# bistromath/gr-ais

Hardware: AMD Instinct MI355X
Metric: complex MS/s through corr_est->msk_timing chain; corr_est %HBM roofline (higher is better)
Workload: dtype f32

## Files before the change

gr-ais_amd/csrc/aisx_common.h:

```cpp
#pragma once
#include <math.h>
#include <stdint.h>

#if defined(__HIPCC__)
#include <hip/hip_runtime.h>
#define AISX_DI __device__ __forceinline__
#define AISX_HD __host__ __device__ __forceinline__
#else
#define AISX_DI inline
#define AISX_HD inline
#endif

namespace aisx {

struct cf {
    float re, im;
};

AISX_HD cf mk(float re, float im)
{
    cf r;
    r.re = re;
    r.im = im;
    return r;
}
AISX_HD cf operator+(cf a, cf b) { return mk(a.re + b.re, a.im + b.im); }
AISX_HD cf operator-(cf a, cf b) { return mk(a.re - b.re, a.im - b.im); }
AISX_HD cf cconj(cf a) { return mk(a.re, -a.im); }

struct alignas(8) cf_a8 { float re, im; };
struct alignas(16) cf_a16 { float re0, im0, re1, im1; };
AISX_HD cf ld8(const cf* p)
{
    const cf_a8 v = *reinterpret_cast<const cf_a8*>(p);
    return mk(v.re, v.im);
}
AISX_HD void st8(cf* p, cf v)
{
    cf_a8 t;
    t.re = v.re;
    t.im = v.im;
    *reinterpret_cast<cf_a8*>(p) = t;
}
AISX_HD void ld16(const cf* p, cf& a, cf& b)
{
    const cf_a16 v = *reinterpret_cast<const cf_a16*>(p);
    a = mk(v.re0, v.im0);
    b = mk(v.re1, v.im1);
}
AISX_HD void st16(cf* p, cf a, cf b)
{
    cf_a16 t;
    t.re0 = a.re;
    t.im0 = a.im;
    t.re1 = b.re;
    t.im1 = b.im;
    *reinterpret_cast<cf_a16*>(p) = t;
}

AISX_HD cf cmul_exact(cf a, cf b) { return mk(a.re * b.re - a.im * b.im, a.re * b.im + a.im * b.re); }

AISX_HD cf cmul_fma(cf a, cf b)
{
    return mk(fmaf(-a.im, b.im, a.re * b.re), fmaf(a.im, b.re, a.re * b.im));
}
AISX_HD cf cmul_conj_fma(cf a, cf b)
{
    return mk(fmaf(a.im, b.im, a.re * b.re), fmaf(a.im, b.re, -(a.re * b.im)));
}

AISX_HD float mag2(cf a) { return a.re * a.re + a.im * a.im; }

AISX_HD float fdiv_rn(float a, float b)
{
#if defined(__HIP_DEVICE_COMPILE__)
    return __fdiv_rn(a, b);
#else
    return a / b;
#endif
}

AISX_HD float branchless_clip(float x, float clip)
{
    float x1 = fabsf(x + clip);
    float x2 = fabsf(x - clip);
    x1 -= x2;
    return 0.5f * x1;
}

AISX_HD int aisx_popc64(unsigned long long v) { return __builtin_popcountll(v); }

AISX_HD unsigned mmse_row_bits(float mu) { return __builtin_bit_cast(unsigned, fmaf(mu, 128.0f, 12582912.0f)); }
AISX_HD unsigned mmse_row(float mu) { return mmse_row_bits(mu) - 0x4B400000u; }
AISX_HD unsigned mmse_row_base(unsigned base, unsigned pitch) { return base - 0x400000u * pitch; }
AISX_HD unsigned mmse_row_off(float mu, unsigned pitch, unsigned row_base)
{
    return (mmse_row_bits(mu) & 0xFFFFFFu) * pitch + row_base;
}

AISX_HD unsigned ring_read_off(int sb, int adv, unsigned step, unsigned mask)
{
#if defined(__HIP_DEVICE_COMPILE__)
    unsigned r;
    asm("v_mad_u32_u24 %0, %1, %2, %3" : "=v"(r) : "v"(adv), "v"(step), "v"(sb));
    return r & mask;
#else
    return ((unsigned)sb + ((unsigned)adv & 0xFFFFFFu) * (step & 0xFFFFFFu)) & mask;
#endif
}

AISX_HD float fast_atan2f_tab(float y, float x, const float* tab)
{
    const float TAN_MAP_RES = 0.003921569f;
    const float PI_F = 3.14159265358979323846f, PI2_F = 1.57079632679489661923f;
    const float y_abs = fabsf(y), x_abs = fabsf(x);
    const bool ylt = y_abs < x_abs;
    const float z = fdiv_rn(ylt ? y_abs : x_abs, ylt ? x_abs : y_abs);
    float alpha = z * 255.0f;
    const int index = ((int)alpha) & 0xff;
    alpha -= (float)index;
    const float t0 = tab[index], t1 = tab[index + 1];
    float base_angle = t0 + (t1 - t0) * alpha;
    base_angle = (z < TAN_MAP_RES) ? z : base_angle;
    const bool xge = x >= 0.0f, yge = y >= 0.0f;
    const float a_h = xge ? (yge ? base_angle : -base_angle) : (yge ? (PI_F - base_angle) : (base_angle - PI_F));
    const float a_v = yge ? (xge ? (PI2_F - base_angle) : (PI2_F + base_angle))
                          : (xge ? (-PI2_F + base_angle) : (-PI2_F - base_angle));
    const float angle = (x_abs > y_abs) ? a_h : a_v;
    return ((y_abs > 0.0f) || (x_abs > 0.0f)) ? angle : 0.0f;
}

AISX_HD int fxpt_float_to_fixed(float x)
{
    const float PI = 3.14159265358979323846f, TAU = 2.0f * 3.14159265358979323846f, TWO_TO_THE_31 = 2147483648.0f;
    if (!(x >= -PI && x < PI)) {
        const int d = (int)floor((double)fdiv_rn(x, TAU) + 0.5);
        x -= (float)d * TAU;
    }
    const float RCP_PI = 0.318309886183790671538f;
    const float y = x * TWO_TO_THE_31;
    const float q = y * RCP_PI;
    return (int)fmaf(fmaf(-q, PI, y), RCP_PI, q);
}
AISX_HD void nco_sincos(float phase, const float* tab, float* s, float* c)
{
    const cf* T = reinterpret_cast<const cf*>(tab);
    const unsigned x = (unsigned)fxpt_float_to_fixed(phase);
    const unsigned xc = x + 0x40000000u;
    const cf es = ld8(T + (x >> 22)), ec = ld8(T + (xc >> 22));
    *s = es.re * (float)(x >> 1) + es.im;
    *c = ec.re * (float)(xc >> 1) + ec.im;
}

AISX_HD float nco_wrap(float ph)
{
    const float F_PI = 3.14159265358979323846f;
    const float TWO_PI = 2.0f * F_PI;
    const float u = ph + F_PI;
    float r;
    const float au = fabsf(u);
    if (au < TWO_PI)
        r = u;
    else if (au < 2.0f * TWO_PI)
        r = (u > 0.f) ? (u - TWO_PI) : (u + TWO_PI);
    else
        r = fmodf(u, TWO_PI);
    return r - F_PI;
}

AISX_HD float nco_wrap_small(float ph)
{
    const float F_PI = 3.14159265358979323846f;
    const float TWO_PI = 2.0f * F_PI;
    const float u = ph + F_PI;
    const float w = u - copysignf(TWO_PI, u);
    const float r = (fabsf(u) < TWO_PI) ? u : w;
    return r - F_PI;
}

#ifndef NCO_CKN
#define NCO_CKN 8
#endif
constexpr int NCO_CK = NCO_CKN;
static_assert(NCO_CK == 2 || NCO_CK == 4 || NCO_CK == 8, "checkpoints every 2, 4 or 8 items");
AISX_HD float nco_phase_step(float ph, float d, bool small) { return small ? nco_wrap_small(ph + d) : nco_wrap(ph + d); }

constexpr int NCO_TAB_FLOATS = 2048;

AISX_HD float cabs_f(cf a) { return (float)sqrt((double)a.re * (double)a.re + (double)a.im * (double)a.im); }

struct tag_rec {
    uint64_t offset;
    double value;
    int32_t key;
    int32_t chan;
};
enum { KEY_CORR_START = 0, KEY_PHASE_EST = 1, KEY_TIME_EST = 2, KEY_CORR_EST = 3 };

}
```

gr-ais_amd/csrc/k_msk.h:

```cpp
#pragma once
#include "aisx_common.h"

namespace aisx {

enum {
    MSK_ST_INTERP_RANGE = 1,
    MSK_ST_CARRY_OVERFLOW = 2,
    MSK_ST_TAGCARRY_OVERFLOW = 4,
    MSK_ST_OUT_FULL = 8,
    MSK_ST_TAGS_TRUNCATED = 16
};
constexpr int MSK_CTN_TRUNC = 0x40000000;
constexpr int MSK_CTN_WILD = 0x20000000;
constexpr int MSK_TAG_TRIPS = 6;

constexpr int MSK_T = 64;
constexpr int MSK_RING = 256;
constexpr int MSK_SLOTS = MSK_RING + 8;
constexpr int MSK_CHUNK = 64;
constexpr int MSK_OFF = 192;
constexpr int MSK_CARRY_MAX = 128;
constexpr int MSK_PAIRS_MAX = 16;
constexpr int MSK_TAPS_PITCH = 12;
constexpr int msk_lds_ring(int lpw) { return MSK_SLOTS * lpw * 8; }
constexpr int MSK_ZERO_ROW = 129;
constexpr int MSK_LDS_MMSE = ((130 * MSK_TAPS_PITCH * 4 + 511) / 512) * 512;
constexpr int MSK_TAGQ = 36;
#ifndef MSK_WAVES_LPW4
#define MSK_WAVES_LPW4 4
#endif
constexpr int msk_waves(int lpw) { return lpw >= 16 ? 64 / lpw : (lpw == 4 ? MSK_WAVES_LPW4 : 4); }
constexpr int msk_wg_channels(int lpw) { return msk_waves(lpw) * lpw; }
constexpr int MSK_STAGE = 32;
static_assert(MSK_STAGE >= 15 + MSK_PAIRS_MAX + 1, "a lock-step run and a general step between two flushes");
constexpr bool msk_staged(int lpw) { return lpw <= 8; }
constexpr int msk_lds_stage(int lpw) { return msk_staged(lpw) ? MSK_STAGE * lpw * 8 : 0; }
constexpr int msk_lds_ringoff(int lpw) { return msk_waves(lpw) * msk_lds_stage(lpw); }
constexpr int msk_lds_wave(int lpw) { return msk_lds_ring(lpw) + MSK_TAGQ * lpw * 8 + lpw * 8; }
constexpr int msk_lds_taboff(int lpw) { return msk_lds_ringoff(lpw) + msk_waves(lpw) * msk_lds_wave(lpw); }
constexpr int msk_lds_bytes(int lpw) { return msk_lds_taboff(lpw) + MSK_LDS_MMSE; }
static_assert(msk_lds_bytes(4) <= 160 * 1024 && msk_lds_bytes(8) <= 160 * 1024 && msk_lds_bytes(16) <= 160 * 1024 &&
              msk_lds_bytes(32) <= 160 * 1024 && msk_lds_bytes(64) <= 160 * 1024, "a workgroup's LDS");
static_assert(msk_lds_bytes(8) + 71680 <= 160 * 1024, "timing recovery + one correlator workgroup per CU");
constexpr int BT_T = 256;
constexpr int BT_SEG = BT_T * 8;

constexpr int MSKP_SMAX = 64;
enum { MSKP_KIND_NONE = 0, MSKP_KIND_NEXT = 1, MSKP_KIND_HANDOFF = 2 };
struct mskp_rst {
    int jA;
    int relA, relB;
    int q0, cap;
    int pad[3];
};
struct mskp_snap {
    int a;
    float mu, omega;
    int div;
    cf y;
    cf nl;
    int cur;
    int cnt;
};
struct mskp_res {
    mskp_snap end;
    cf ay, anl;
    int kind;
    int status;
};
struct mskp_piece {
    int out0, src0, cnt;
};
AISX_HD bool mskp_same_bits(cf a, cf b)
{
    unsigned ar, ai, br, bi;
    __builtin_memcpy(&ar, &a.re, 4);
    __builtin_memcpy(&ai, &a.im, 4);
    __builtin_memcpy(&br, &b.re, 4);
    __builtin_memcpy(&bi, &b.im, 4);
    return ar == br && ai == bi;
}

struct msk_ctag { int rel; float val; };

struct __attribute__((packed, aligned(8))) cf_pair { cf a, b; };

struct MskParams {
    int nchan;
    float d_sps, gain, gain_omega, limit;
    int osps;
    float* mu; float* omega; int* div;
    cf* dly1; cf* dly2; cf* diff1;
    unsigned long long* nread;
    const cf* in; long in_stride; int n;
    const cf* carry_in; cf* carry_out; const int* carry_len_in; int* carry_len_out; int carry_cap;
    int stream_mode; int gr_ninput; int gr_noutput;
    const msk_ctag* ct; const int* ct_n; int ct_cap;
    tag_rec* ctag_out; int* ctag_n_out; int ctag_cap;
    cf* syms; float* err; float* mu_out; long out_stride; int out_cap;
    int* produced; int* consumed; int* status;
    const float* mmse;
    int lds_tab_off;
    int lds_wave_stride, tq_stride, tq_private;
    int lds_ring_off;
    int sym_al16;
    int lpw;
    int inline_tags;
    int max_noutput;
    int ff;
    const int* nrst; const mskp_rst* rst; const mskp_res* res;
    mskp_piece* pieces; int* npieces;
    const int* ct_nc;
};

struct BitTailParams {
    int nchan;
    const cf* syms; long sym_stride;
    const int* produced;
    unsigned char* bits; long bit_stride;
    const cf* prev_sym_in; const unsigned char* prev_bit_in;
    cf* prev_sym_out; unsigned char* prev_bit_out;
    const float* atan_tab;
};

AISX_HD int msk_forecast(float d_sps, int noutput_items)
{
    return (int)ceil((noutput_items * d_sps * 2) + 3.0 * d_sps + 8u);
}

#ifdef MSK_EMU_STATS
extern long msk_stats[8];
#endif
template <class Ctx, bool AUX, bool OSPS2, int LPW, bool FFT = false>
AISX_DI void msk_body(Ctx& cx, const MskParams& p)
{
    static_assert(!FFT || (!AUX && !OSPS2), "the join build has no err / mu ports and osps == 1");
    constexpr int SLOT_B = LPW * 8;
    constexpr int SLOT_SH = LPW == 64 ? 9 : (LPW == 32 ? 8 : (LPW == 16 ? 7 : (LPW == 8 ? 6 : 5)));
    static_assert(LPW == 4 || LPW == 8 || LPW == 16 || LPW == 32 || LPW == 64, "channels per wave");
    typedef unsigned long long u64;
    static_assert(64 % LPW == 0, "whole waves");
    constexpr int NQ = 64 / LPW;
    constexpr int QS = MSK_CHUNK / NQ;
    const int wv = cx.tid() >> 6;
    const int l = cx.tid() & (LPW - 1);
    const int q = (cx.tid() & 63) / LPW;
    const bool owner = q == 0;
    const int cbase = cx.bx() * msk_wg_channels(LPW) + wv * LPW;
    const int c = cbase + l;
    const bool live = c < p.nchan;
    const int cc = live ? c : (p.nchan - 1);

    char* const lds0 = cx.lds();
    char* const lds = lds0 + p.lds_ring_off + wv * p.lds_wave_stride;
    cf* ring = (cf*)lds;
    float* mm = (float*)(lds0 + p.lds_tab_off);
    cf* myring = ring + l;

    for (int i = cx.tid(); i < 129 * 8; i += cx.nthreads())
        mm[(i >> 3) * MSK_TAPS_PITCH + (i & 7)] = p.mmse[i];
    if (cx.tid() < MSK_TAPS_PITCH)
        mm[MSK_ZERO_ROW * MSK_TAPS_PITCH + cx.tid()] = 0.f;
    if (cbase >= p.nchan) {
        cx.sync();
        return;
    }

    const float d_sps = p.d_sps;
    float d_mu = p.mu[cc], d_omega = p.omega[cc];
    int d_div = p.div[cc];
    cf last_interp = p.dly1[cc];
    cf d_dly_diff_1 = p.diff1[cc];
    cf prev_sq = cmul_exact(p.dly2[cc], p.dly2[cc]);
    const unsigned long long R = p.nread[cc];
    int status = 0;
    const int n = p.n;

    const cf* cin = p.carry_in + (long)cc * p.carry_cap;
    int pending = p.carry_len_in[cc];
    if (pending > MSK_CARRY_MAX)
        pending = MSK_CARRY_MAX;
    const int navail = pending + n;
    for (int q = -1; q < pending; q++) {
        const int slot = (q - pending + MSK_OFF) & (MSK_RING - 1);
        myring[slot * LPW] = cin[q + 1];
        if (slot < 8)
            myring[(MSK_RING + slot) * LPW] = cin[q + 1];
    }

    const msk_ctag* ctl = p.ct + (long)cc * p.ct_cap;
    int ntot = p.ct_n[cc];
    if (ntot & MSK_CTN_TRUNC)
        status |= MSK_ST_TAGS_TRUNCATED;
    const bool tame_tags = p.inline_tags && cx.ballot((ntot & MSK_CTN_WILD) != 0) == 0ull;
    ntot &= MSK_CTN_WILD - 1;
    if (ntot > p.ct_cap)
        ntot = p.ct_cap;
    typedef msk_ctag tq_ent;
    tq_ent* const tq = (tq_ent*)(lds + msk_lds_ring(LPW)) + (p.tq_private ? (cx.tid() & 63) : l);
    const int TQS = p.tq_stride;
    const int TQ_NONE = 0x7fffffff;
    int gq = 0;
    int qhead = 0, qn = 0;
    auto tq_fill = [&]() {
        if (qn > 0) {
            tq[0] = tq[(qn - 1) * TQS];
            qn = 1;
        }
        qhead = qn;
        while (qn < MSK_TAGQ && gq < ntot) {
            tq_ent t[4];
#pragma unroll
            for (int j = 0; j < 4; j++)
                t[j] = ctl[gq + j < ntot ? gq + j : ntot - 1];
#pragma unroll
            for (int j = 0; j < 4; j++) {
                if (qn < MSK_TAGQ && gq < ntot) {
                    gq++;
                    tq[qn * TQS] = t[j];
                    qn++;
                }
            }
        }
    };
    int fr_rel = TQ_NONE;
    float nt_val = 0.f;
    int nt_rel = 0x7fffffff;
    auto tq_front = [&]() {
        if (qhead >= qn && gq < ntot)
            tq_fill();
        if (qhead < qn) {
            const tq_ent e = tq[qhead * TQS];
            fr_rel = e.rel;
            nt_val = e.val;
        } else {
            fr_rel = TQ_NONE;
        }
    };
    auto tq_pop = [&]() {
        qhead++;
        tq_front();
    };
    tq_fill();

    constexpr bool FF = FFT;
    bool fin_saved = false;
    float fin_mu = 0.f, fin_omega = 0.f;
    int fin_div = 0, fin_status = 0;
    cf fin_interp = mk(0.f, 0.f), fin_diff = mk(0.f, 0.f);
    unsigned fin_worst = 0;
    int ffK = 0, ffnck = 0, cand = 0, candj = 0x7fffffff, ffnp = 0;
    int voff = 0;
    const mskp_rst* const ffrs = FF ? p.rst + (long)cc * MSKP_SMAX : nullptr;
    const mskp_res* const ffrr = FF ? p.res + (long)cc * MSKP_SMAX : nullptr;
    if (FF) {
        ffnck = p.ct_nc[cc];
        ffK = ffnck >= 0 ? p.nrst[cc] : 0;
        candj = ffK > 0 ? ffrs[0].jA + 1 + ffnck : 0x7fffffff;
    }

    char* const osym0 = (char*)(p.syms + (long)cbase * p.out_stride);
    char* const oerr0 = AUX && p.err ? (char*)(p.err + (long)cbase * p.out_stride) : nullptr;
    char* const omu0 = AUX && p.mu_out ? (char*)(p.mu_out + (long)cbase * p.out_stride) : nullptr;
    unsigned ob = (unsigned)((long)(cc - cbase) * p.out_stride) * 8u;
    constexpr bool STG = !AUX && !OSPS2 && msk_staged(LPW);
    constexpr unsigned FLQ = NQ < 8 ? NQ : 8;
    constexpr unsigned FL = 2 * FLQ;
    constexpr unsigned STG_MASK = (unsigned)((MSK_STAGE - 1) * SLOT_B);
    const unsigned obrow = ob;
    const unsigned stg_real = (unsigned)(wv * msk_lds_stage(LPW) + l * 8);
    const unsigned stg_spare = (unsigned)(p.lds_ring_off + wv * p.lds_wave_stride + p.lds_wave_stride - SLOT_B + l * 8);
    unsigned so = 0;
    unsigned nf = 0;
    struct alignas(8) cf8s { float re, im; };
    auto stage_put = [&](unsigned mask, unsigned base, cf v) {
        cf8s t;
        t.re = v.re;
        t.im = v.im;
        *(cf8s*)(lds0 + ((so & mask) | base)) = t;
        so += (unsigned)SLOT_B;
    };
    auto stage_get = [&](unsigned k) -> cf {
        const cf8s t = *(const cf8s*)(lds0 + ((((k & (unsigned)(MSK_STAGE - 1)) << SLOT_SH)) | stg_real));
        return mk(t.re, t.im);
    };
    auto flush_syms = [&]() {
        if constexpr (STG) {
            if (cx.ballot((so >> SLOT_SH) - nf >= FL) == 0ull)
                return;
            cx.wave_sync();
            while (cx.ballot((so >> SLOT_SH) - nf >= FL) != 0ull) {
                if ((so >> SLOT_SH) - nf >= FL) {
                    const unsigned k0 = nf + 2u * (unsigned)q;
                    if ((NQ <= 8 || (unsigned)q < FLQ) && !fin_saved) {
                        const cf a = stage_get(k0), b = stage_get(k0 + 1u);
                        cf* dst = (cf*)(osym0 + obrow) + k0;
                        if (p.sym_al16) {
                            st16(dst, a, b);
                        } else {
                            st8(dst, a);
                            st8(dst + 1, b);
                        }
                    }
                    nf += FL;
                }
            }
            cx.wave_sync();
        }
    };

    int base = 0, ototal = 0;
    int iidx = 0, oidx = 0;
    int ninp = 0, noutput = 0;
// ... 128 lines not shown
            ffnp++;
            moved = true;
            dcnt += r.end.cnt;
            oidx_w += r.end.cnt;
            while (p.max_noutput > 0 && oidx_w >= nout_w) {
                oidx_w -= nout_w;
                otot_w += nout_w;
                nout_w = p.max_noutput;
                crossed = true;
            }
            a_new = r.end.a;
            mu_new = r.end.mu;
            om_new = r.end.omega;
            div_new = r.end.div;
            yv = r.end.y;
            nlv = r.end.nl;
            cur_new = r.end.cur;
            status |= r.status;
            cand++;
            candj = cand < ffK ? ffrs[cand].jA + 1 + ffnck : 0x7fffffff;
            if (r.kind == MSKP_KIND_NEXT && cand < ffK)
                continue;
            break;
        }
        if (!moved)
            return false;
        if constexpr (STG) {
            if (owner) {
                for (unsigned kk = nf; kk < (so >> SLOT_SH); kk++)
                    st8((cf*)(osym0 + obrow) + kk, stage_get(kk));
            }
            nf = (so >> SLOT_SH) + (unsigned)dcnt;
            so += (unsigned)dcnt << SLOT_SH;
        }
        ob += (unsigned)dcnt * 8u;
        d_mu = mu_new;
        d_omega = om_new;
        d_div = div_new;
        last_interp = yv;
        prev_sq = cmul_exact(yv, yv);
        d_dly_diff_1 = nlv;
        gq = cur_new + ffnck;
        if (gq > ntot)
            gq = ntot;
        qn = 0;
        qhead = 0;
        tq_fill();
        const int q_new = a_new + pending;
        tq_front();
        if (crossed) {
            ototal = otot_w;
            base = (fr_rel != TQ_NONE && fr_rel < q_new) ? fr_rel : q_new;
            setup_round();
        } else {
            nt_rel = (fr_rel != TQ_NONE && fr_rel - base < ninp) ? fr_rel - base : 0x7fffffff;
        }
        iidx = q_new - base;
        oidx = oidx_w;
        const int v_new = loaded_s - MSK_CHUNK + 1;
        voff = a_new - v_new;
        sb = (v_new + MSK_OFF) * SLOT_B;
        {
            const int slot0 = (loaded_s - MSK_CHUNK + MSK_OFF) & (MSK_RING - 1);
            constexpr int SH = Ctx::wave_lds_coherent ? 1 : NQ;
            for (int sh = 0; sh < SH; sh++) {
                const int k0 = ((Ctx::wave_lds_coherent ? q : sh) * QS);
                cf t[QS];
#pragma unroll
                for (int k = 0; k < QS; k++) {
                    const int sr = loaded_s - MSK_CHUNK + k0 + k + voff;
                    t[k] = mk(0.f, 0.f);
                    if (sr >= 0 && sr < n)
                        t[k] = myin[sr];
                }
#pragma unroll
                for (int k = 0; k < QS; k++) {
                    myring[(slot0 + k0 + k) * LPW] = t[k];
                    if (slot0 == 0 && k0 + k < 8)
                        myring[(MSK_RING + k0 + k) * LPW] = t[k];
                }
            }
            if (more) {
                const int s0 = landed * MSK_CHUNK + q * QS + voff;
#pragma unroll
                for (int k = 0; k < QS; k++) {
                    r[k] = mk(0.f, 0.f);
                    if (s0 + k < n && s0 + k >= 0)
                        r[k] = myin[s0 + k];
                }
            }
        }
        tag_trig = (int)0x80000000;
        fast_lim = (int)0x80000000;
        return true;
    };
    auto events = [&](const int PAR) -> int {
        if (!(oidx < noutput && iidx < ninp)) {
            base += iidx;
            ototal += oidx;
            const bool progress = iidx > 0;
            if (!p.stream_mode || !progress)
                done = true;
            else
                setup_round();
        }
        if (done)
            return EV_PARK;
        const int spos = sb >> SLOT_SH;
        const bool waiting = more && !(spos - MSK_OFF + 8 + jump_margin <= loaded_s);
        if (!waiting && (nt_rel >= iidx) && ((float)nt_rel < ((float)iidx + d_sps))) {
            if (FF) {
                const int fi = gq - (qn - qhead);
                while (cand < ffK && candj < fi) {
                    cand++;
                    candj = cand < ffK ? ffrs[cand].jA + 1 + ffnck : 0x7fffffff;
                }
                if (cand < ffK && fi == candj && ff_walk()) {
                    bounds(sb >> SLOT_SH);
                    return EV_OTHER_PARITY;
                }
            }
            const float center = nt_val;
            if (center == center) {
                const int old = iidx;
                d_mu = center;
                iidx = nt_rel;
                if (d_mu < 0) {
                    d_mu++;
                    iidx--;
                }
                sb += (iidx - old) * SLOT_B;
                d_div = 0;
                d_omega = d_sps;
            }
            tq_pop();
            nt_rel = (fr_rel != TQ_NONE && fr_rel - base < ninp) ? fr_rel - base : 0x7fffffff;
            bounds(sb >> SLOT_SH);
            if (fast_lim <= iidx) {
                tag_trig = TRIG_FORCED;
                fast_lim = iidx + 1;
            }
            return ((d_div & 1) == PAR) ? EV_GO : EV_OTHER_PARITY;
        }
        bounds(spos);
        if (waiting)
            return EV_PARK;
        return EV_GO;
    };

    auto tap_row = [&](float mu) -> unsigned {
        const unsigned imu = (unsigned)(int)rintf(mu * 128.0f);
        return imu < (unsigned)MSK_ZERO_ROW ? imu : (unsigned)MSK_ZERO_ROW;
    };
    auto fir_load = [&](unsigned row, int sbpos, cf* sv, float* tv) {
        typedef float tap4 __attribute__((vector_size(16)));
        const tap4* tp4 = (const tap4*)((const char*)mm + row * (unsigned)(MSK_TAPS_PITCH * 4));
        const tap4 tlo = tp4[0], thi = tp4[1];
        const float tp[8] = { tlo[0], tlo[1], tlo[2], tlo[3], thi[0], thi[1], thi[2], thi[3] };
        struct alignas(8) cf8 { float re, im; };
        const cf8* sp = (const cf8*)(lds + (((unsigned)sbpos & (unsigned)((MSK_RING - 1) * SLOT_B)) | (unsigned)(l * 8)));
#pragma unroll
        for (int k = 0; k < 8; k++) {
            const cf8 t = sp[k * LPW];
            sv[k] = mk(t.re, t.im);
            tv[k] = tp[7 - k];
        }
    };
    const unsigned mm_rbase = mmse_row_base((unsigned)p.lds_tab_off, (unsigned)(MSK_TAPS_PITCH * 4));
    const char* const lds_l = lds + l * 8;
    constexpr unsigned RING_M = (unsigned)((MSK_RING - 1) * SLOT_B);
    auto fir_load_pair = [&](float mu, unsigned soff, cf* sv, float* tv) {
        typedef float tap4 __attribute__((vector_size(16)));
        const tap4* tp4 = (const tap4*)(lds0 + mmse_row_off(mu, (unsigned)(MSK_TAPS_PITCH * 4), mm_rbase));
        const tap4 tlo = tp4[0], thi = tp4[1];
        const float tp[8] = { tlo[0], tlo[1], tlo[2], tlo[3], thi[0], thi[1], thi[2], thi[3] };
        struct alignas(8) cf8 { float re, im; };
        const cf8* sp = (const cf8*)(lds_l + soff);
#pragma unroll
        for (int k = 0; k < 8; k++) {
            const cf8 t = sp[k * LPW];
            sv[k] = mk(t.re, t.im);
            tv[k] = tp[7 - k];
        }
    };
    auto fir_sum = [&](const cf* sv, const float* tv) -> cf {
        cf acc = mk(0.f, 0.f);
#pragma unroll
        for (int k = 0; k < 8; k++) {
            acc.re += sv[k].re * tv[k];
            acc.im += sv[k].im * tv[k];
        }
        return acc;
    };

    auto fir = [&](unsigned row, int sbpos) -> cf {
        cf sv[8];
        float tv[8];
        fir_load(row, sbpos, sv, tv);
        return fir_sum(sv, tv);
    };

    auto body = [&](const int PAR) {
        const unsigned row = tap_row(d_mu);
        worst_imu = worst_imu > row ? worst_imu : row;
        const cf in_interp = fir(row, sb);
        const cf sq = cmul_exact(in_interp, in_interp);
        const cf dly_conj = cconj(prev_sq);
        const cf nlin_out = cmul_exact(sq, dly_conj);
        float err_out = (nlin_out - d_dly_diff_1).re;
        if (PAR) {
            err_out = branchless_clip(err_out, 3.0f);
            d_omega += p.gain_omega * err_out;
            d_omega = d_sps + branchless_clip(d_omega - d_sps, p.limit);
            d_mu += p.gain * err_out;
        }
        if (!PAR || OSPS2) {
            if constexpr (STG)
                stage_put(STG_MASK, stg_real, in_interp);
            else
                *(cf*)(osym0 + ob) = in_interp;
            if (AUX) {
                if (oerr0)
                    *(float*)(oerr0 + (ob >> 1)) = err_out;
                if (omu0)
                    *(float*)(omu0 + (ob >> 1)) = d_mu;
            }
            ob += 8u;
            oidx++;
        }
        d_div++;
        last_interp = in_interp;
        prev_sq = sq;
        d_dly_diff_1 = nlin_out;
        d_mu += d_omega;
        const float fl = floorf(d_mu);
        const int adv = (int)fl;
        iidx += adv;
        sb += adv * SLOT_B;
        d_mu = d_mu - fl;
    };

#ifdef MSK_PROF
    long long pf_t0 = __builtin_readcyclecounter(), pf_lock = 0, pf_land = 0, pf_gen = 0, pf_n[4] = {0, 0, 0, 0}, pf_fail = 0, pf_nfail = 0;
#define PF_BEGIN long long pf_a = __builtin_readcyclecounter();
#define PF_END(acc) acc += __builtin_readcyclecounter() - pf_a;
#else
#define PF_BEGIN
#define PF_END(acc)
#endif
    u64 P = 0;
    u64 E = 0;
    auto ok_for = [&](const int PAR) -> bool {
        return (PAR || OSPS2) ? ((iidx < fast_lim) && (oidx < noutput)) : (iidx < fast_lim);
    };

    auto step = [&](const int PAR) {
        const u64 mine = ~P & (PAR ? ~E : E);
        const u64 okM = cx.ballot(ok_for(PAR));
        u64 goM = mine & okM;
        const u64 evM = mine & ~okM;
        if (evM != 0ull) {
#ifdef MSK_PROF
            pf_n[3]++;
#endif
            int code = -1;
            if (cx.inv_ballot(evM))
                code = events(PAR);
            goM |= cx.ballot(code == EV_GO);
            P |= cx.ballot(code == EV_PARK);
            E = cx.ballot((d_div & 1) == 0);
        }
        if (goM != 0ull) {
            if (cx.inv_ballot(goM))
                body(PAR);
            E ^= goM;
        }
    };

    const u64 ALL = cx.ballot(true);

    const float wmax = d_sps + fabsf(p.limit);
    const float pair_adv = 2.0f * wmax + 3.0f * fabsf(p.gain);
    const float pair_adv_inv = 0.9999f / pair_adv;
    const bool lock_ok = 3.0f * fabsf(p.gain) + fabsf(p.limit) + 0.01f < d_sps;
    auto rearm = [&]() {
        const int chunk_lim = more ? (loaded_s - 8 - jump_margin + MSK_OFF - ((sb >> SLOT_SH) - iidx) + 1) : 0x7fffffff;
        int f = ninp < tag_trig ? ninp : tag_trig;
        f = f < chunk_lim ? f : chunk_lim;
        fast_lim = (tag_trig == TRIG_FORCED) ? fast_lim : f;
    };
    auto need_more = [&]() -> bool {
        return FF ? cx.ballot(!done && landed * MSK_CHUNK < n + 8 - voff) != 0ull : landed < nchunks;
    };
    more = need_more();
    if (more)
        issue_chunk(landed);
    loaded_s = landed * MSK_CHUNK;
    P = cx.ballot(done);
    E = cx.ballot((d_div & 1) == 0);
    rearm();
    for (;;) {
        flush_syms();
        const u64 DN = FF ? cx.ballot(done) : 0ull;
        if (FF && done && !fin_saved) {
            fin_saved = true;
            fin_mu = d_mu;
            fin_omega = d_omega;
            fin_div = d_div;
            fin_interp = last_interp;
            fin_diff = d_dly_diff_1;
            fin_status = status;
            fin_worst = worst_imu;
            if constexpr (STG) {
                if (owner) {
                    for (unsigned kk = nf; kk < (so >> SLOT_SH); kk++)
                        st8((cf*)(osym0 + obrow) + kk, stage_get(kk));
                }
                nf = so >> SLOT_SH;
            }
        }
        { PF_BEGIN
        if ((P & ~DN) == 0ull && (E | DN) == ALL && DN != ALL) {
            const float room = fast_lim > iidx ? (float)(fast_lim - iidx) - (1.001f + wmax) : -1.f;
            int can = room >= 0.f ? (int)(room * pair_adv_inv) + 1 : 0;
            can = can < MSK_PAIRS_MAX ? can : MSK_PAIRS_MAX;
            const int ocan = OSPS2 ? (noutput - oidx) / 2 : (noutput - oidx) - 1;
            can = can < ocan ? can : ocan;
            if (!lock_ok || !(d_mu >= 0.f && d_mu <= 1.f))
                can = 0;
            int npairs = 0;
            if ((cx.ballot(can >= 1) | DN) == ALL) {
                npairs = MSK_PAIRS_MAX;
                if ((cx.ballot(can >= MSK_PAIRS_MAX) | DN) != ALL) {
                    npairs = 1;
                    for (int bit = MSK_PAIRS_MAX / 2; bit; bit >>= 1)
                        if (npairs + bit < MSK_PAIRS_MAX && (cx.ballot(can >= npairs + bit) | DN) == ALL)
                            npairs += bit;
                }
            }
            if constexpr (NQ >= 2 && !AUX && !OSPS2) {
              if (npairs == 0 && tame_tags) {
                constexpr int ROW = LPW <= 16 ? 16 : 32;
                const int chunk_lim2 = more ? (loaded_s - 8 - jump_margin + MSK_OFF - ((sb >> SLOT_SH) - iidx) + 1) : 0x7fffffff;
                const int lim2 = ninp < chunk_lim2 ? ninp : chunk_lim2;
                const float room2 = lim2 > iidx ? (float)(lim2 - iidx) - (1.001f + wmax + d_sps) : -1.f;
                int can2 = room2 >= 0.f ? (int)(room2 * (0.9999f / (pair_adv + d_sps))) + 1 : 0;
                can2 = can2 < MSK_TAG_TRIPS ? can2 : MSK_TAG_TRIPS;
                can2 = can2 < ocan ? can2 : ocan;
                if (!lock_ok || !(d_mu >= 0.f && d_mu <= 1.f) || tag_trig == TRIG_FORCED)
                    can2 = 0;
                int ntrips = 0;
                if ((cx.ballot(can2 >= 1) | DN) == ALL) {
                    ntrips = 1;
                    while (ntrips < MSK_TAG_TRIPS && (cx.ballot(can2 >= ntrips + 1) | DN) == ALL)
                        ntrips++;
                }
                if (ntrips > 0) {
                    const bool roleO = (cx.tid() & ROW) != 0;
                    const unsigned rstep = (unsigned)(cx.tid() & ROW) * (unsigned)(SLOT_B / ROW);
                    const unsigned pmask = roleO ? 0u : STG_MASK, pbase = roleO ? stg_spare : stg_real;
                    cf sqO = prev_sq, sqE = mk(0.f, 0.f), acc = last_interp;
                    float nl_prev = d_dly_diff_1.re;
                    bool last_skip = false;
                    for (int k = 0; k < ntrips; k++) {
#ifdef MSK_EMU_STATS
                        if (l == 0 && q == 0) msk_stats[5]++;
#endif
                        const bool fireE = (nt_rel >= iidx) && ((float)nt_rel < ((float)iidx + d_sps));
                        if (cx.ballot(fireE) != 0ull) {
                            if (fireE) {
                                const float center = nt_val;
                                if (center == center) {
                                    int at = nt_rel;
                                    float m = center;
                                    if (m < 0) {
                                        m++;
                                        at--;
                                    }
                                    sb += (at - iidx) * SLOT_B;
                                    iidx = at;
                                    d_mu = m;
                                    d_div = 0;
                                    d_omega = d_sps;
                                }
                                tq_pop();
                                nt_rel = (fr_rel != TQ_NONE && fr_rel - base < ninp) ? fr_rel - base : 0x7fffffff;
                            }
                        }
                        const float m1 = d_mu + d_omega;
                        const float muO = cx.fract(m1);
                        const int adv1 = (int)m1;
                        const int sb1 = sb + adv1 * SLOT_B;
                        const int iidxO = iidx + adv1;
                        const bool winO = (nt_rel >= iidxO) && ((float)nt_rel < ((float)iidxO + d_sps));
                        const bool nanO = winO && (nt_val != nt_val);
                        if (cx.ballot(nanO) != 0ull) {
                            if (nanO) {
                                tq_pop();
                                nt_rel = (fr_rel != TQ_NONE && fr_rel - base < ninp) ? fr_rel - base : 0x7fffffff;
                            }
                        }
                        const bool skipO = winO && !nanO;
                        cf sv[8];
                        float tv[8];
                        fir_load_pair(roleO ? muO : d_mu, ring_read_off(sb, adv1, rstep, RING_M), sv, tv);
                        acc = fir_sum(sv, tv);
                        const cf sq = cmul_exact(acc, acc);
                        cf sE, s1;
                        cx.template pair_rows<ROW>(sq, sE, s1);
                        const float nlE = sE.re * sqO.re + sE.im * sqO.im;
                        const float nlO = s1.re * sE.re + s1.im * sE.im;
                        const float err = branchless_clip(nlO - nlE, 3.0f);
                        float om2 = d_omega + p.gain_omega * err;
                        om2 = d_sps + branchless_clip(om2 - d_sps, p.limit);
                        const float mu2 = muO + p.gain * err;
                        if constexpr (STG) {
                            stage_put(pmask, pbase, acc);
                        } else {
                            if (!roleO)
                                *(cf*)(osym0 + ob) = acc;
                            ob += 8u;
                        }
                        const float m2 = mu2 + om2;
                        const int adv2 = (int)m2;
                        d_mu = skipO ? muO : cx.fract(m2);
                        sb = skipO ? sb1 : sb1 + adv2 * SLOT_B;
                        iidx = skipO ? iidxO : iidxO + adv2;
                        d_omega = skipO ? d_omega : om2;
                        d_div += skipO ? 1 : 2;
                        const cf nE = skipO ? sqO : sE, nO = skipO ? sE : s1;
                        sqE = nE;
                        sqO = nO;
                        nl_prev = skipO ? nlE : nlO;
                        last_skip = skipO;
                    }
                    cf accE, accO;
                    cx.template pair_rows<ROW>(acc, accE, accO);
                    oidx += ntrips;
                    prev_sq = sqO;
                    last_interp = last_skip ? accE : accO;
                    d_dly_diff_1 = mk(nl_prev, sqO.im * sqE.re - sqO.re * sqE.im);
                    if (!(d_mu >= 0.f && d_mu <= 1.f))
                        status |= MSK_ST_INTERP_RANGE;
                    E = cx.ballot((d_div & 1) == 0);
                    bounds(sb >> SLOT_SH);
#ifdef MSK_PROF
                    pf_n[0] += ntrips; pf_n[1]++;
#endif
                }
              }
            }
#ifdef MSK_PROF
            if (npairs == 0) { pf_fail += __builtin_readcyclecounter() - pf_a; pf_nfail++; }
#endif
            if (npairs > 0) {
              if constexpr (NQ >= 2) {
                constexpr int ROW = LPW <= 16 ? 16 : 32;
                const bool roleO = (cx.tid() & ROW) != 0;
                const unsigned rstep = (unsigned)(cx.tid() & ROW) * (unsigned)(SLOT_B / ROW);
                const unsigned pmask = roleO ? 0u : STG_MASK, pbase = roleO ? stg_spare : stg_real;
                cf sqO = prev_sq, sqE = mk(0.f, 0.f), acc = last_interp;
                float nl_prev = d_dly_diff_1.re;
                const int sb_entry = sb;
                for (int k = 0; k < npairs; k++) {
#ifdef MSK_EMU_STATS
                    if (l == 0 && q == 0) msk_stats[0]++;
#endif
                    const float m1 = d_mu + d_omega;
                    const float muO = cx.fract(m1);
                    const int adv1 = (int)m1;
                    const int sb1 = sb + adv1 * SLOT_B;
                    cf sv[8];
                    float tv[8];
                    fir_load_pair(roleO ? muO : d_mu, ring_read_off(sb, adv1, rstep, RING_M), sv, tv);
                    acc = fir_sum(sv, tv);
                    const cf sq = cmul_exact(acc, acc);
                    cf sE, s1;
                    cx.template pair_rows<ROW>(sq, sE, s1);
                    const float nlE = sE.re * sqO.re + sE.im * sqO.im;
                    const float nlO = s1.re * sE.re + s1.im * sE.im;
                    const float err = branchless_clip(nlO - nlE, 3.0f);
                    d_omega += p.gain_omega * err;
                    d_omega = d_sps + branchless_clip(d_omega - d_sps, p.limit);
                    const float mu2 = muO + p.gain * err;
                    if (OSPS2) {
                        const unsigned o = ob + (roleO ? 8u : 0u);
                        *(cf*)(osym0 + o) = acc;
                        if (AUX) {
                            if (oerr0)
                                *(float*)(oerr0 + (o >> 1)) = roleO ? err : nlE - nl_prev;
                            if (omu0)
                                *(float*)(omu0 + (o >> 1)) = roleO ? mu2 : d_mu;
                        }
                        ob += 16u;
                    } else if constexpr (STG) {
                        stage_put(pmask, pbase, acc);
                    } else {
                        if (!roleO) {
                            *(cf*)(osym0 + ob) = acc;
                            if (AUX) {
                                if (oerr0)
                                    *(float*)(oerr0 + (ob >> 1)) = nlE - nl_prev;
                                if (omu0)
                                    *(float*)(omu0 + (ob >> 1)) = d_mu;
                            }
                        }
                        ob += 8u;
                    }
                    const float m2 = mu2 + d_omega;
                    d_mu = cx.fract(m2);
                    sb = sb1 + (int)m2 * SLOT_B;
                    sqE = sE;
                    sqO = s1;
                    nl_prev = nlO;
                }
                cf accE, accO;
                cx.template pair_rows<ROW>(acc, accE, accO);
                d_div += 2 * npairs;
                oidx += OSPS2 ? 2 * npairs : npairs;
                iidx += (sb - sb_entry) >> SLOT_SH;
                prev_sq = sqO;
                last_interp = accO;
                d_dly_diff_1 = mk(nl_prev, sqO.im * sqE.re - sqO.re * sqE.im);
                if (!(d_mu >= 0.f && d_mu <= 1.f))
                    status |= MSK_ST_INTERP_RANGE;
              } else {
                const int sb_entry = sb;
                cf sqO = prev_sq, sqE = mk(0.f, 0.f), accO = last_interp;
                float nl_prev = d_dly_diff_1.re;
                for (int k = 0; k < npairs; k++) {
#ifdef MSK_EMU_STATS
                    if (l == 0) msk_stats[0]++;
#endif
                    cf svE[8], svO[8];
                    float tvE[8], tvO[8];
                    fir_load_pair(d_mu, (unsigned)sb & RING_M, svE, tvE);
                    const float m1 = d_mu + d_omega;
                    const float muO = cx.fract(m1);
                    const int sb1 = sb + (int)m1 * SLOT_B;
                    fir_load_pair(muO, (unsigned)sb1 & RING_M, svO, tvO);
                    const cf accE = fir_sum(svE, tvE);
                    const cf sE = cmul_exact(accE, accE);
                    const float nlE = sE.re * sqO.re + sE.im * sqO.im;
                    if constexpr (STG)
                        stage_put(STG_MASK, stg_real, accE);
                    else
                        *(cf*)(osym0 + ob) = accE;
                    if (AUX) {
                        if (oerr0)
                            *(float*)(oerr0 + (ob >> 1)) = nlE - nl_prev;
                        if (omu0)
                            *(float*)(omu0 + (ob >> 1)) = d_mu;
                    }
                    ob += 8u;
                    const cf acc1 = fir_sum(svO, tvO);
                    const cf s1 = cmul_exact(acc1, acc1);
                    const float nlO = s1.re * sE.re + s1.im * sE.im;
                    const float err = branchless_clip(nlO - nlE, 3.0f);
                    d_omega += p.gain_omega * err;
                    d_omega = d_sps + branchless_clip(d_omega - d_sps, p.limit);
                    const float mu2 = muO + p.gain * err;
                    if (OSPS2) {
                        *(cf*)(osym0 + ob) = acc1;
                        if (AUX) {
                            if (oerr0)
                                *(float*)(oerr0 + (ob >> 1)) = err;
                            if (omu0)
                                *(float*)(omu0 + (ob >> 1)) = mu2;
                        }
                        ob += 8u;
                    }
                    const float m2 = mu2 + d_omega;
                    d_mu = cx.fract(m2);
                    sb = sb1 + (int)m2 * SLOT_B;
                    sqE = sE;
                    sqO = s1;
                    accO = acc1;
                    nl_prev = nlO;
                }
                d_div += 2 * npairs;
                oidx += OSPS2 ? 2 * npairs : npairs;
                iidx += (sb - sb_entry) >> SLOT_SH;
                prev_sq = sqO;
                last_interp = accO;
                d_dly_diff_1 = mk(nl_prev, sqO.im * sqE.re - sqO.re * sqE.im);
                if (!(d_mu >= 0.f && d_mu <= 1.f))
                    status |= MSK_ST_INTERP_RANGE;
              }
#ifdef MSK_PROF
                pf_n[0] += npairs; pf_n[1]++;
#endif
            }
        }
        PF_END(pf_lock) }
        { PF_BEGIN
        if (FF && !more) {
            more = need_more();
            if (more)
                issue_chunk(landed);
        }
        if (more) {
            const bool clear = done || ((sb >> SLOT_SH) - MSK_OFF >= landed * MSK_CHUNK - (MSK_RING - MSK_CHUNK) + 2);
            if (cx.ballot(clear) == ALL) {
#ifdef MSK_EMU_STATS
                if (l == 0) msk_stats[4]++;
#endif
                cx.wave_sync();
                land_chunk(landed);
                cx.wave_sync();
                landed++;
                more = need_more();
                if (more)
                    issue_chunk(landed);
                loaded_s = landed * MSK_CHUNK;
                P = cx.ballot(done);
                rearm();
                if (P == 0ull && E == ALL) {
                    PF_END(pf_land)
                    continue;
                }
            }
        }
        PF_END(pf_land) }
#ifdef MSK_EMU_STATS
        if (l == 0) { msk_stats[1]++; if (P != 0ull) msk_stats[2]++; if (E != ALL && E != 0ull) msk_stats[3]++; }
#endif
        { PF_BEGIN
        step(0);
        step(1);
#ifdef MSK_PROF
        pf_n[2]++;
#endif
        PF_END(pf_gen) }
        if (P == ALL && (!more || cx.ballot(done) == ALL))
            break;
    }

#ifdef MSK_PROF
    if (c == 0 && owner) {
        long long pf_t1 = __builtin_readcyclecounter();
        printf("msk prof: total %lld lock %lld (failed entries %lld: %lld) land %lld gen %lld | pairs %lld runs %lld genpasses %lld events %lld\n", pf_t1 - pf_t0, pf_lock, pf_nfail, pf_fail, pf_land, pf_gen, pf_n[0], pf_n[1], pf_n[2], pf_n[3]);
    }
#endif
    if constexpr (STG) {
        flush_syms();
        const unsigned left = fin_saved ? 0u : (so >> SLOT_SH) - nf;
#pragma unroll
        for (unsigned j = 0; j < 2; j++) {
            const unsigned k = (unsigned)q + j * FLQ;
            if ((unsigned)q < FLQ && k < left)
                st8((cf*)(osym0 + obrow) + nf + k, stage_get(nf + k));
        }
    }
    if (!live || !owner)
        return;
    if (fin_saved) {
        d_mu = fin_mu;
        d_omega = fin_omega;
        d_div = fin_div;
        last_interp = fin_interp;
        d_dly_diff_1 = fin_diff;
        status = fin_status;
        worst_imu = fin_worst;
    }
    if (worst_imu >= (unsigned)MSK_ZERO_ROW)
        status |= MSK_ST_INTERP_RANGE;
    p.mu[c] = d_mu;
    p.omega[c] = d_omega;
    p.div[c] = d_div;
    p.dly1[c] = last_interp;
    p.dly2[c] = last_interp;
    p.diff1[c] = d_dly_diff_1;
    const unsigned long long Rn = R + (unsigned long long)base;
    p.nread[c] = Rn;
    p.produced[c] = ototal;
    p.consumed[c] = base;

    cf* cout = p.carry_out + (long)c * p.carry_cap;
    if (p.stream_mode) {
        int left = navail - base;
        int cap = p.carry_cap < MSK_CARRY_MAX ? p.carry_cap : MSK_CARRY_MAX;
        if (left + 1 > cap) {
            status |= MSK_ST_CARRY_OVERFLOW;
            left = cap - 1;
        }
        if (FF) {
            for (int k = 0; k <= left; k++) {
                const int qi = base - 1 + k;
                cout[k] = qi < pending ? cin[qi + 1] : myin[qi - pending];
            }
            p.npieces[c] = ffnp;
        } else {
            for (int k = 0; k <= left; k++)
                cout[k] = myring[((base - 1 + k - pending + MSK_OFF) & (MSK_RING - 1)) * LPW];
        }
        p.carry_len_out[c] = left;
        tag_rec* cto = p.ctag_out + (long)c * p.ctag_cap;
        int w = 0;
        for (int k = 0; k < qn; k++) {
            const tq_ent e = tq[k * TQS];
            if (e.rel < base)
                continue;
            if (w < p.ctag_cap) {
                tag_rec tg;
                tg.offset = R + (unsigned long long)e.rel;
                tg.value = (double)e.val;
                tg.key = KEY_TIME_EST;
                tg.chan = c;
                cto[w] = tg;
            } else {
                status |= MSK_ST_TAGCARRY_OVERFLOW;
            }
            w++;
        }
        for (int k = gq; k < ntot; k++) {
            const tq_ent e = ctl[k];
            if (e.rel < base)
                continue;
            if (w < p.ctag_cap) {
                tag_rec tg;
                tg.offset = R + (unsigned long long)e.rel;
                tg.value = (double)e.val;
                tg.key = KEY_TIME_EST;
                tg.chan = c;
                cto[w] = tg;
            } else {
                status |= MSK_ST_TAGCARRY_OVERFLOW;
            }
            w++;
        }
        p.ctag_n_out[c] = w < p.ctag_cap ? w : p.ctag_cap;
    } else {
        cout[0] = myring[((base - 1 - pending + MSK_OFF) & (MSK_RING - 1)) * LPW];
        p.carry_len_out[c] = 0;
        p.ctag_n_out[c] = 0;
    }
    p.status[c] = status;
}

struct TagPrepParams {
    int nchan;
    const tag_rec* ctag_in; const int* ctag_n_in; int ctag_cap;
    const tag_rec* tags; const int* tag_count; int tag_cap;
    const unsigned long long* nread;
    msk_ctag* ct; int* ct_n; int ct_cap;
    int* ct_nc;
    const msk_ctag* ctl_new; const int* ctl_new_n; int ctl_new_cap; int ctl_new_pre; unsigned long long W;
};

template <class Ctx>
AISX_DI void tagprep_body(Ctx& cx, const TagPrepParams& p)
{
    const int l = cx.tid() & 63;
    const int c = cx.bx() * (cx.nthreads() >> 6) + (cx.tid() >> 6);
    if (c >= p.nchan)
        return;
    const unsigned long long R = p.nread[c];
    msk_ctag* out = p.ct + (long)c * p.ct_cap;
    int w = 0;
    bool wild = false;
    auto scan = [&](const tag_rec* list, int n) {
        for (int k0 = 0; k0 < n; k0 += 64) {
            const int k = k0 + l;
            tag_rec t;
            t.offset = 0;
            t.value = 0;
            t.key = -1;
            if (k < n)
                t = list[k];
            const bool keep = (k < n) && t.key == KEY_TIME_EST && t.offset >= R;
            const float tv = (float)t.value;
            if (cx.ballot(keep && !(tv != tv) && !(tv >= -1.0f && tv <= 1.0f)) != 0ull)
                wild = true;
            const unsigned long long m = cx.ballot(keep);
            const int pos = w + aisx_popc64(m & ((1ull << l) - 1ull));
            if (keep && pos < p.ct_cap) {
                const unsigned long long d = t.offset - R;
                msk_ctag e;
                e.rel = d > 0x7ffffff0ull ? 0x7ffffff0 : (int)d;
                e.val = (float)t.value;
                out[pos] = e;
            }
            w += aisx_popc64(m);
        }
    };
    bool trunc = false;
    int nc = p.ctag_n_in[c];
    if (nc > p.ctag_cap)
        nc = p.ctag_cap;
    scan(p.ctag_in + (long)c * p.ctag_cap, nc);
    const int kept_carried = w;
    bool newdrop = false;
    if (p.ctl_new) {
        int nn = p.ctl_new_n[c];
// ... 105 lines not shown
```

Before: 47930.

## Reorder MMSE FIR LDS loads, store taps reversed, use packed f32 math

Stores the MMSE tap table in reversed order within each row so the FIR no longer needs a per-load tap reversal. Splits the FIR sample and tap loads into interleaved groups separated by scheduling barriers, so the ring reads can issue before the tap-row address is ready. Replaces the scalar FIR sum, complex square and dot products with packed v_pk f32 math, and uses permlane swaps instead of the previous row-pairing shuffle. It also adds optional per-pair cycle profiling. The scheduling barriers may constrain the compiler, and the inline asm adds correctness risk.

```diff
diff --git a/gr-ais_amd/csrc/aisx_common.h b/gr-ais_amd/csrc/aisx_common.h
--- a/gr-ais_amd/csrc/aisx_common.h
+++ b/gr-ais_amd/csrc/aisx_common.h
@@ -106,6 +106,93 @@
     return r & mask;
 #else
     return ((unsigned)sb + ((unsigned)adv & 0xFFFFFFu) * (step & 0xFFFFFFu)) & mask;
+#endif
+}
+
+AISX_HD unsigned mmse_tab_slot(unsigned i, unsigned pitch_floats) { return (i >> 3) * pitch_floats + (7u - (i & 7u)); }
+AISX_HD unsigned mmse_tab_row_off(unsigned row, unsigned pitch_bytes) { return row * pitch_bytes; }
+
+AISX_HD void sched_fence()
+{
+#if defined(__HIP_DEVICE_COMPILE__)
+    __builtin_amdgcn_sched_barrier(0);
+#endif
+}
+#if defined(__HIP_DEVICE_COMPILE__)
+typedef float pk2f __attribute__((ext_vector_type(2)));
+#endif
+typedef float aisx_tap4 __attribute__((vector_size(16)));
+AISX_HD cf fir8_sum(const cf* s, aisx_tap4 tlo, aisx_tap4 thi)
+{
+#if defined(__HIP_DEVICE_COMPILE__)
+    pk2f acc = { 0.f, 0.f };
+#pragma unroll
+    for (int k = 0; k < 8; k++) {
+        const aisx_tap4 h = k < 4 ? tlo : thi;
+        const pk2f t = { h[k & 2], h[(k & 2) + 1] }, a = { s[k].re, s[k].im };
+        acc = acc + a * ((k & 1) ? t.yy : t.xx);
+    }
+    return mk(acc.x, acc.y);
+#else
+    const float t[8] = { tlo[0], tlo[1], tlo[2], tlo[3], thi[0], thi[1], thi[2], thi[3] };
+    cf acc = mk(0.f, 0.f);
+    for (int k = 0; k < 8; k++) {
+        acc.re += s[k].re * t[k];
+        acc.im += s[k].im * t[k];
+    }
+    return acc;
+#endif
+}
+AISX_HD void csq_exact2(cf a, cf& s0, cf& s1)
+{
+#if defined(__HIP_DEVICE_COMPILE__)
+    const pk2f av = { a.re, a.im };
+    pk2f p, q, r0, r1;
+    asm("v_pk_mul_f32 %0, %1, %1 op_sel:[1,1] op_sel_hi:[0,1]" : "=v"(q) : "v"(av));
+    asm("v_pk_mul_f32 %0, %1, %1 op_sel_hi:[1,0]" : "=v"(p) : "v"(av));
+    asm("v_pk_add_f32 %0, %1, %2 neg_lo:[0,1]" : "=v"(r0) : "v"(p), "v"(q));
+    asm("v_pk_add_f32 %0, %1, %2 neg_lo:[0,1] ; second set" : "=v"(r1) : "v"(p), "v"(q));
+    s0 = mk(r0.x, r0.y);
+    s1 = mk(r1.x, r1.y);
+#else
+    s0 = s1 = cmul_exact(a, a);
+#endif
+}
+
+AISX_HD void pair_nl_re(cf sE, cf s1, cf sqO, float& nlE, float& nlO)
+{
+#if defined(__HIP_DEVICE_COMPILE__)
+    const pk2f e = { sE.re, sE.im }, o = { s1.re, s1.im }, d = { sqO.re, sqO.im };
+    const pk2f a = e * d, b = o * e;
+    nlE = a.x + a.y;
+    nlO = b.x + b.y;
+#else
+    nlE = sE.re * sqO.re + sE.im * sqO.im;
+    nlO = s1.re * sE.re + s1.im * sE.im;
+#endif
+}
+
+template <int W, class Ctx>
+AISX_DI void pair_rows2(const Ctx& cx, cf v0, cf v1, cf& lo, cf& hi)
+{
+#if defined(__HIP_DEVICE_COMPILE__)
+    static_assert(W == 16 || W == 32, "row width");
+    const unsigned a0 = __builtin_bit_cast(unsigned, v0.re), b0 = __builtin_bit_cast(unsigned, v0.im);
+    const unsigned a1 = __builtin_bit_cast(unsigned, v1.re), b1 = __builtin_bit_cast(unsigned, v1.im);
+    if constexpr (W == 16) {
+        const auto ra = __builtin_amdgcn_permlane16_swap(a0, a1, false, false);
+        const auto rb = __builtin_amdgcn_permlane16_swap(b0, b1, false, false);
+        lo = mk(__builtin_bit_cast(float, (unsigned)ra[0]), __builtin_bit_cast(float, (unsigned)rb[0]));
+        hi = mk(__builtin_bit_cast(float, (unsigned)ra[1]), __builtin_bit_cast(float, (unsigned)rb[1]));
+    } else {
+        const auto ra = __builtin_amdgcn_permlane32_swap(a0, a1, false, false);
+        const auto rb = __builtin_amdgcn_permlane32_swap(b0, b1, false, false);
+        lo = mk(__builtin_bit_cast(float, (unsigned)ra[0]), __builtin_bit_cast(float, (unsigned)rb[0]));
+        hi = mk(__builtin_bit_cast(float, (unsigned)ra[1]), __builtin_bit_cast(float, (unsigned)rb[1]));
+    }
+#else
+    (void)v1;
+    cx.template pair_rows<W>(v0, lo, hi);
 #endif
 }
 
diff --git a/gr-ais_amd/csrc/k_msk.h b/gr-ais_amd/csrc/k_msk.h
--- a/gr-ais_amd/csrc/k_msk.h
+++ b/gr-ais_amd/csrc/k_msk.h
@@ -158,7 +158,7 @@
     cf* myring = ring + l;
 
     for (int i = cx.tid(); i < 129 * 8; i += cx.nthreads())
-        mm[(i >> 3) * MSK_TAPS_PITCH + (i & 7)] = p.mmse[i];
+        mm[mmse_tab_slot((unsigned)i, MSK_TAPS_PITCH)] = p.mmse[i];
     if (cx.tid() < MSK_TAPS_PITCH)
         mm[MSK_ZERO_ROW * MSK_TAPS_PITCH + cx.tid()] = 0.f;
     if (cbase >= p.nchan) {
@@ -593,52 +593,53 @@
         const unsigned imu = (unsigned)(int)rintf(mu * 128.0f);
         return imu < (unsigned)MSK_ZERO_ROW ? imu : (unsigned)MSK_ZERO_ROW;
     };
-    auto fir_load = [&](unsigned row, int sbpos, cf* sv, float* tv) {
-        typedef float tap4 __attribute__((vector_size(16)));
-        const tap4* tp4 = (const tap4*)((const char*)mm + row * (unsigned)(MSK_TAPS_PITCH * 4));
-        const tap4 tlo = tp4[0], thi = tp4[1];
-        const float tp[8] = { tlo[0], tlo[1], tlo[2], tlo[3], thi[0], thi[1], thi[2], thi[3] };
-        struct alignas(8) cf8 { float re, im; };
+    typedef aisx_tap4 tap4;
+    struct alignas(8) cf8 { float re, im; };
+    auto tap_read = [&](unsigned tab_byte_off, int half) -> tap4 {
+        return ((const tap4*)(lds0 + tab_byte_off))[half];
+    };
+    auto ring_read2 = [&](const cf8* sp, int k, cf* sv) {
+        const cf8 t0 = sp[k * LPW], t1 = sp[(k + 1) * LPW];
+        sv[k] = mk(t0.re, t0.im);
+        sv[k + 1] = mk(t1.re, t1.im);
+    };
+    auto fir_load = [&](unsigned row, int sbpos, cf* sv, tap4& tlo, tap4& thi) {
+        const unsigned toff = (unsigned)p.lds_tab_off + mmse_tab_row_off(row, (unsigned)(MSK_TAPS_PITCH * 4));
+        tlo = tap_read(toff, 0);
+        thi = tap_read(toff, 1);
         const cf8* sp = (const cf8*)(lds + (((unsigned)sbpos & (unsigned)((MSK_RING - 1) * SLOT_B)) | (unsigned)(l * 8)));
 #pragma unroll
-        for (int k = 0; k < 8; k++) {
-            const cf8 t = sp[k * LPW];
-            sv[k] = mk(t.re, t.im);
-            tv[k] = tp[7 - k];
-        }
+        for (int k = 0; k < 8; k += 2)
+            ring_read2(sp, k, sv);
     };
     const unsigned mm_rbase = mmse_row_base((unsigned)p.lds_tab_off, (unsigned)(MSK_TAPS_PITCH * 4));
     const char* const lds_l = lds + l * 8;
     constexpr unsigned RING_M = (unsigned)((MSK_RING - 1) * SLOT_B);
-    auto fir_load_pair = [&](float mu, unsigned soff, cf* sv, float* tv) {
-        typedef float tap4 __attribute__((vector_size(16)));
-        const tap4* tp4 = (const tap4*)(lds0 + mmse_row_off(mu, (unsigned)(MSK_TAPS_PITCH * 4), mm_rbase));
-        const tap4 tlo = tp4[0], thi = tp4[1];
-        const float tp[8] = { tlo[0], tlo[1], tlo[2], tlo[3], thi[0], thi[1], thi[2], thi[3] };
-        struct alignas(8) cf8 { float re, im; };
+    auto fir_load_first = [&](unsigned soff, cf* sv) -> const cf8* {
         const cf8* sp = (const cf8*)(lds_l + soff);
-#pragma unroll
-        for (int k = 0; k < 8; k++) {
-            const cf8 t = sp[k * LPW];
-            sv[k] = mk(t.re, t.im);
-            tv[k] = tp[7 - k];
-        }
-    };
-    auto fir_sum = [&](const cf* sv, const float* tv) -> cf {
-        cf acc = mk(0.f, 0.f);
-#pragma unroll
-        for (int k = 0; k < 8; k++) {
-            acc.re += sv[k].re * tv[k];
-            acc.im += sv[k].im * tv[k];
-        }
-        return acc;
-    };
+        ring_read2(sp, 0, sv);
+        sched_fence();
+        return sp;
+    };
+    auto fir_load_rest = [&](float mu, const cf8* sp, cf* sv, tap4& tlo, tap4& thi) {
+        const unsigned toff = mmse_row_off(mu, (unsigned)(MSK_TAPS_PITCH * 4), mm_rbase);
+        tlo = tap_read(toff, 0);
+        sched_fence();
+        ring_read2(sp, 2, sv);
+        sched_fence();
+        thi = tap_read(toff, 1);
+        sched_fence();
+        ring_read2(sp, 4, sv);
+        ring_read2(sp, 6, sv);
+        sched_fence();
+    };
+    auto fir_sum = [&](const cf* sv, tap4 tlo, tap4 thi) -> cf { return fir8_sum(sv, tlo, thi); };
 
     auto fir = [&](unsigned row, int sbpos) -> cf {
         cf sv[8];
-        float tv[8];
-        fir_load(row, sbpos, sv, tv);
-        return fir_sum(sv, tv);
+        tap4 tlo, thi;
+        fir_load(row, sbpos, sv, tlo, thi);
+        return fir_sum(sv, tlo, thi);
     };
 
     auto body = [&](const int PAR) {
@@ -685,9 +686,26 @@
     long long pf_t0 = __builtin_readcyclecounter(), pf_lock = 0, pf_land = 0, pf_gen = 0, pf_n[4] = {0, 0, 0, 0}, pf_fail = 0, pf_nfail = 0;
 #define PF_BEGIN long long pf_a = __builtin_readcyclecounter();
 #define PF_END(acc) acc += __builtin_readcyclecounter() - pf_a;
+    long long pf_sec[3] = {0, 0, 0}, pf_npl = 0;
+#define PF_PAIR_TOP const long long pf_p0 = __builtin_readcyclecounter();
+#define PF_PAIR_ISSUED                                              \
+    const long long pf_p1 = __builtin_readcyclecounter();            \
+    asm volatile("s_waitcnt lgkmcnt(0)" ::: "memory");              \
+    const long long pf_p2 = __builtin_readcyclecounter();
+#define PF_PAIR_END                                                 \
+    {                                                               \
+        const long long pf_p3 = __builtin_readcyclecounter();       \
+        pf_sec[0] += pf_p1 - pf_p0;                                 \
+        pf_sec[1] += pf_p2 - pf_p1;                                 \
+        pf_sec[2] += pf_p3 - pf_p2;                                 \
+        pf_npl++;                                                   \
+    }
 #else
 #define PF_BEGIN
 #define PF_END(acc)
+#define PF_PAIR_TOP
+#define PF_PAIR_ISSUED
+#define PF_PAIR_END
 #endif
     u64 P = 0;
     u64 E = 0;
@@ -843,14 +861,16 @@
                         }
                         const bool skipO = winO && !nanO;
                         cf sv[8];
-                        float tv[8];
-                        fir_load_pair(roleO ? muO : d_mu, ring_read_off(sb, adv1, rstep, RING_M), sv, tv);
-                        acc = fir_sum(sv, tv);
-                        const cf sq = cmul_exact(acc, acc);
+                        tap4 tlo, thi;
+                        const cf8* sp = fir_load_first(ring_read_off(sb, adv1, rstep, RING_M), sv);
+                        fir_load_rest(roleO ? muO : d_mu, sp, sv, tlo, thi);
+                        acc = fir_sum(sv, tlo, thi);
+                        cf sq, sq2;
+                        csq_exact2(acc, sq, sq2);
                         cf sE, s1;
-                        cx.template pair_rows<ROW>(sq, sE, s1);
-                        const float nlE = sE.re * sqO.re + sE.im * sqO.im;
-                        const float nlO = s1.re * sE.re + s1.im * sE.im;
+                        pair_rows2<ROW>(cx, sq, sq2, sE, s1);
+                        float nlE, nlO;
+                        pair_nl_re(sE, s1, sqO, nlE, nlO);
                         const float err = branchless_clip(nlO - nlE, 3.0f);
                         float om2 = d_omega + p.gain_omega * err;
                         om2 = d_sps + branchless_clip(om2 - d_sps, p.limit);
@@ -907,19 +927,23 @@
 #ifdef MSK_EMU_STATS
                     if (l == 0 && q == 0) msk_stats[0]++;
 #endif
+                    PF_PAIR_TOP
                     const float m1 = d_mu + d_omega;
+                    const int adv1 = (int)m1;
+                    cf sv[8];
+                    tap4 tlo, thi;
+                    const cf8* sp = fir_load_first(ring_read_off(sb, adv1, rstep, RING_M), sv);
                     const float muO = cx.fract(m1);
-                    const int adv1 = (int)m1;
+                    fir_load_rest(roleO ? muO : d_mu, sp, sv, tlo, thi);
+                    PF_PAIR_ISSUED
                     const int sb1 = sb + adv1 * SLOT_B;
-                    cf sv[8];
-                    float tv[8];
-                    fir_load_pair(roleO ? muO : d_mu, ring_read_off(sb, adv1, rstep, RING_M), sv, tv);
-                    acc = fir_sum(sv, tv);
-                    const cf sq = cmul_exact(acc, acc);
+                    acc = fir_sum(sv, tlo, thi);
+                    cf sq, sq2;
+                    csq_exact2(acc, sq, sq2);
                     cf sE, s1;
-                    cx.template pair_rows<ROW>(sq, sE, s1);
-                    const float nlE = sE.re * sqO.re + sE.im * sqO.im;
-                    const float nlO = s1.re * sE.re + s1.im * sE.im;
+                    pair_rows2<ROW>(cx, sq, sq2, sE, s1);
+                    float nlE, nlO;
+                    pair_nl_re(sE, s1, sqO, nlE, nlO);
                     const float err = branchless_clip(nlO - nlE, 3.0f);
                     d_omega += p.gain_omega * err;
                     d_omega = d_sps + branchless_clip(d_omega - d_sps, p.limit);
@@ -954,6 +978,7 @@
                     sqE = sE;
                     sqO = s1;
                     nl_prev = nlO;
+                    PF_PAIR_END
                 }
                 cf accE, accO;
                 cx.template pair_rows<ROW>(acc, accE, accO);
@@ -974,13 +999,15 @@
                     if (l == 0) msk_stats[0]++;
 #endif
                     cf svE[8], svO[8];
-                    float tvE[8], tvO[8];
-                    fir_load_pair(d_mu, (unsigned)sb & RING_M, svE, tvE);
+                    tap4 tloE, thiE, tloO, thiO;
+                    const cf8* spE = fir_load_first((unsigned)sb & RING_M, svE);
+                    fir_load_rest(d_mu, spE, svE, tloE, thiE);
                     const float m1 = d_mu + d_omega;
                     const float muO = cx.fract(m1);
                     const int sb1 = sb + (int)m1 * SLOT_B;
-                    fir_load_pair(muO, (unsigned)sb1 & RING_M, svO, tvO);
-                    const cf accE = fir_sum(svE, tvE);
+                    const cf8* spO = fir_load_first((unsigned)sb1 & RING_M, svO);
+                    fir_load_rest(muO, spO, svO, tloO, thiO);
+                    const cf accE = fir_sum(svE, tloE, thiE);
                     const cf sE = cmul_exact(accE, accE);
                     const float nlE = sE.re * sqO.re + sE.im * sqO.im;
                     if constexpr (STG)
@@ -994,7 +1021,7 @@
                             *(float*)(omu0 + (ob >> 1)) = d_mu;
                     }
                     ob += 8u;
-                    const cf acc1 = fir_sum(svO, tvO);
+                    const cf acc1 = fir_sum(svO, tloO, thiO);
                     const cf s1 = cmul_exact(acc1, acc1);
                     const float nlO = s1.re * sE.re + s1.im * sE.im;
                     const float err = branchless_clip(nlO - nlE, 3.0f);
@@ -1080,7 +1107,7 @@
 #ifdef MSK_PROF
     if (c == 0 && owner) {
         long long pf_t1 = __builtin_readcyclecounter();
-        printf("msk prof: total %lld lock %lld (failed entries %lld: %lld) land %lld gen %lld | pairs %lld runs %lld genpasses %lld events %lld\n", pf_t1 - pf_t0, pf_lock, pf_nfail, pf_fail, pf_land, pf_gen, pf_n[0], pf_n[1], pf_n[2], pf_n[3]);
+        printf("msk prof: total %lld lock %lld (failed entries %lld: %lld) land %lld gen %lld | pairs %lld runs %lld genpasses %lld events %lld | plain pairs %lld, their sections: to last read issued %lld, to all reads returned %lld, rest %lld\n", pf_t1 - pf_t0, pf_lock, pf_nfail, pf_fail, pf_land, pf_gen, pf_n[0], pf_n[1], pf_n[2], pf_n[3], pf_npl, pf_sec[0], pf_sec[1], pf_sec[2]);
     }
 #endif
     if constexpr (STG) {
```

New measurement: 48230, median of 6. About the same (+0.6%).
